# PJLab-ADG/DetZero

Hardware: AMD Instinct MI355X
Metric: LiDAR frames/sec (160k pts, 0.1m voxels) (higher is better)
Workload: dtype f32 as f16 pairs (hi+lo, 22-bit significand; 3 f16 MFMA per product, f32 accumulate)

## Files before the change

### detzero_amd/csrc/conv2d_h.hip

```cpp
#include "hgemm.h"

namespace dz {

int conv3x3_h_variant(const dz_conv2d_desc &p);
int conv3x3_h_launch(const dz_conv2d_desc &p, int bc, int math, int out_f32, size_t w_bytes, hipStream_t stream);

template <class T, class M, bool OUT_F32, int NS>
__global__ __launch_bounds__(256) void k_conv2d_h(dz_conv2d_desc p, long m_total, unsigned int in_bytes, unsigned int w_bytes) {
    extern __shared__ __attribute__((aligned(16))) unsigned char smem_raw[];
    v4u *const smem = reinterpret_cast<v4u *>(smem_raw);
    __shared__ int in_pix[T::BP];
    __shared__ int out_pix[T::BP];
    __shared__ __attribute__((aligned(16))) float sc_s[T::BC], sh_s[T::BC];

    const int tid = threadIdx.x, lane = tid & 63, wid = tid >> 6;
    const int wp = wid / T::WC, wc = wid % T::WC;
    const int ntn = p.cout_pad / T::BC;
    const int nty = ntn * p.groups;
    const int nwg = gridDim.x, q8 = nwg >> 3, r8 = nwg & 7, xcd = blockIdx.x & 7;
    const int lid = (xcd < r8 ? xcd * (q8 + 1) : r8 * (q8 + 1) + (xcd - r8) * q8) + (blockIdx.x >> 3);
    const int by = lid % nty;
    const int grp = by / ntn;
    const int n0 = (by % ntn) * T::BC;
    const long row0 = (long)(lid / nty) * T::BP;
    const bool phases = p.phase_groups != 0;
    const int ph_dy = phases ? grp / p.out_sx : 0, ph_dx = phases ? grp % p.out_sx : 0;
    const int ssg = phases ? 0 : grp;

// ... 163 lines not shown
                }
            }
        }
    }
}

template <class T, class M, bool OUT_F32, int NS>
static int launch_conv_h(const dz_conv2d_desc &p, size_t w_bytes, hipStream_t stream) {
    const long m_total = (long)p.batch * p.ho * p.wo;
    dim3 grid(ceil_div(m_total, T::BP) * (p.cout_pad / T::BC) * p.groups);
    const size_t in_bytes = (size_t)p.batch * p.in_hp * p.in_wp * p.in_cstride * sizeof(float);
    if (in_bytes >= 0x80000000ull || w_bytes >= 0x80000000ull) {
        set_error("dz_conv2d_forward_split: image of %zu bytes / weights of %zu bytes exceed the 2 GiB buffer-addressing limit", in_bytes, w_bytes);
        return DZ_ERR_UNSUPPORTED;
    }
    static PerDeviceFlags lds_done;
    if (int rc_ = reserve_lds(reinterpret_cast<const void *>(&k_conv2d_h<T, M, OUT_F32, NS>), T::LDS_BYTES, lds_done, "dz_conv2d_forward_split")) return rc_;
    hipLaunchKernelGGL((k_conv2d_h<T, M, OUT_F32, NS>), grid, dim3(256), T::LDS_BYTES, stream, p, m_total, (unsigned int)in_bytes,
                       (unsigned int)w_bytes);
    DZ_LAUNCH_CHECK();
    return DZ_OK;
}

enum ConvHVariant { CH_NONE = 0, CH_128_128, CH_128_64, CH_64_128, CH_64_64, CH_128_32, CH_C3_128, CH_C3_64, CH_C3_32 };
static const char *const kConvHVariantName[] = {"none", "k_conv2d_h<128x128x32>", "k_conv2d_h<128x64x32>", "k_conv2d_h<64x128x32>",
                                                "k_conv2d_h<64x64x32>", "k_conv2d_h<128x32x32>", "k_conv3x3_h<8x32x128>",
                                                "k_conv3x3_h<8x32x64>", "k_conv3x3_h<16x32x32>"};

static ConvHVariant conv2d_h_select(const dz_conv2d_desc &p) {
    if (p.cin % 32 != 0) return CH_NONE;
    const long m_total = (long)p.batch * p.ho * p.wo;
    if (p.cout_pad % 64 != 0) return p.cout_pad % 32 == 0 ? CH_128_32 : CH_NONE;
    struct Cand { ConvHVariant v; int bp, bc; double eff; };
    static const Cand cands[4] = {{CH_128_128, 128, 128, 1.00}, {CH_128_64, 128, 64, 0.90}, {CH_64_128, 64, 128, 0.88}, {CH_64_64, 64, 64, 0.78}};
    const int slots = 512;
    double best = -1.0;
    ConvHVariant pick = CH_64_64;
    for (int i = 0; i < 4; ++i) {
        if (p.cout_pad % cands[i].bc != 0) continue;
        const long tiles = (long)ceil_div(m_total, cands[i].bp) * (p.cout_pad / cands[i].bc) * p.groups;
        const long rounds = (tiles + slots - 1) / slots;
        const double useful = (double)m_total / ((double)ceil_div(m_total, cands[i].bp) * cands[i].bp);
        const double score = cands[i].eff * useful * (double)tiles / (double)(rounds * slots);
        if (score > best) { best = score; pick = cands[i].v; }
    }
    return pick;
}

struct ConvHChoice { ConvHVariant v; const char *why; };

static ConvHChoice conv_h_select(const dz_conv2d_desc &p, int out_f32) {
    const int bc3 = conv3x3_h_variant(p);
    if (p.in_rowidx && (!bc3 || out_f32))
        return {CH_NONE, "dz_conv2d_forward_split: in_rowidx (sparse input) is implemented for 3 x 3 stride-1 layers with 128-channel output tiles, "
                         "two z slabs (cin == 2 * in_row_channels) and pair16 output"};
    if (p.in_tiles && bc3 && !((bc3 == 64 || bc3 == 128) && !out_f32))
        return {CH_NONE, "dz_conv2d_forward_split: in_tiles lists 8 x 32 pixel tiles; this layer runs on the 32-channel tile kernel (16 x 32 tiles) - pass no list"};
    if (bc3 && (!out_f32 || bc3 == 32)) return {bc3 == 128 ? CH_C3_128 : bc3 == 64 ? CH_C3_64 : CH_C3_32, nullptr};
    const ConvHVariant v = conv2d_h_select(p);
    return {v, v != CH_NONE ? nullptr : "dz_conv2d_forward_split: unsupported channels cin=%d cout_pad=%d (cin %% 32, cout_pad %% 32 required)"};
}

template <class M, bool OUT_F32>
static int conv2d_h_launch(ConvHVariant v, const dz_conv2d_desc &p, size_t w_bytes, hipStream_t stream) {
    switch (v) {
        case CH_128_128: return launch_conv_h<HTile<128, 128, 32, 2, 2>, M, OUT_F32, 2>(p, w_bytes, stream);
        case CH_128_64: return launch_conv_h<HTile<128, 64, 32, 2, 2>, M, OUT_F32, 3>(p, w_bytes, stream);
        case CH_64_128: return launch_conv_h<HTile<64, 128, 32, 2, 2>, M, OUT_F32, 3>(p, w_bytes, stream);
        case CH_64_64: return launch_conv_h<HTile<64, 64, 32, 2, 2>, M, OUT_F32, 3>(p, w_bytes, stream);
        default: return launch_conv_h<HTile<128, 32, 32, 4, 1>, M, OUT_F32, 3>(p, w_bytes, stream);
    }
}

}

using namespace dz;

extern "C" {

int dz_conv2d_forward_split(const dz_conv2d_desc *d, int math, int out_f32, void *stream_) {
    hipStream_t stream = (hipStream_t)stream_;
// ... 10 lines not shown
        DZ_CHECK_ARG(d->g_cout[g] >= 1 && d->g_cout[g] <= d->cout_pad, "dz_conv2d_forward_split: bad g_cout[%d]", g);
        DZ_CHECK_ARG(out_f32 || (d->g_cout[g] % 8 == 0 && d->g_ooff[g] % 8 == 0),
                     "dz_conv2d_forward_split: pair16 output needs channel counts / offsets in multiples of 8");
    }
    DZ_CHECK_ARG(out_f32 || (d->out_cstride % 8 == 0 && d->out_coff % 8 == 0),
                 "dz_conv2d_forward_split: pair16 output needs channel stride / offset in multiples of 8");
    DZ_CHECK_ARG((d->ho - 1) * d->stride + d->in_off + d->kh - 1 < d->in_hp &&
                 (d->wo - 1) * d->stride + d->in_off + d->kw - 1 < d->in_wp && d->in_off >= 0,
                 "dz_conv2d_forward_split: taps leave the input image");
    DZ_CHECK_ARG(!d->phase_groups || (d->groups == d->out_sy * d->out_sx && d->kh == 1 && d->kw == 1 && d->stride == 1 && !d->group_shift && !d->group_max),
                 "dz_conv2d_forward_split: phase_groups needs groups == out_sy * out_sx (<= 8) and a 1x1 kernel");
    const int ph_y = d->phase_groups ? d->out_sy - 1 : 0, ph_x = d->phase_groups ? d->out_sx - 1 : 0;
    DZ_CHECK_ARG((d->ho - 1) * d->out_sy + d->out_dy + ph_y < d->out_hp && (d->wo - 1) * d->out_sx + d->out_dx + ph_x < d->out_wp,
                 "dz_conv2d_forward_split: output leaves the output image");
    if ((long)d->batch * d->ho * d->wo == 0) return DZ_OK;
    const size_t w_bytes = (size_t)d->groups * d->kh * d->kw * d->cout_pad * d->cin * sizeof(float);
    DZ_CHECK_ARG(!d->in_rowidx || (d->in_row_channels >= 32 && d->in_rows >= 0), "dz_conv2d_forward_split: in_rowidx needs in_row_channels / in_rows");
    const ConvHChoice c = conv_h_select(*d, out_f32);
    switch (c.v) {
        case CH_NONE: set_error(c.why, d->cin, d->cout_pad); return DZ_ERR_UNSUPPORTED;
        case CH_C3_128: return conv3x3_h_launch(*d, 128, math, out_f32, w_bytes, stream);
        case CH_C3_64: return conv3x3_h_launch(*d, 64, math, out_f32, w_bytes, stream);
        case CH_C3_32: return conv3x3_h_launch(*d, 32, math, out_f32, w_bytes, stream);
        default: break;
    }
    if (math == DZ_MATH_F16X2)
        return out_f32 ? conv2d_h_launch<MathF16, true>(c.v, *d, w_bytes, stream) : conv2d_h_launch<MathF16, false>(c.v, *d, w_bytes, stream);
    if (math == DZ_MATH_F16)
        return out_f32 ? conv2d_h_launch<MathF16H, true>(c.v, *d, w_bytes, stream) : conv2d_h_launch<MathF16H, false>(c.v, *d, w_bytes, stream);
    return out_f32 ? conv2d_h_launch<MathBF16, true>(c.v, *d, w_bytes, stream) : conv2d_h_launch<MathBF16, false>(c.v, *d, w_bytes, stream);
}

int dz_linear_forward_split(const float *x, long rows, int cin, int x_stride, const float *w, int cout, int cout_pad, const float *scale,
                            const float *shift, const float *group_shift, int group_rows, int relu, float *y, int y_stride, int math,
                            int out_f32, int group_max, void *stream_) {
    DZ_CHECK_ARG(rows >= 0 && x_stride >= cin && y_stride >= cout && cin % 32 == 0 && cout_pad % 32 == 0 && cout <= cout_pad,
                 "dz_linear_forward_split: bad sizes (cin and cout_pad in multiples of 32)");
    if (group_max) {
        DZ_CHECK_ARG(out_f32 && group_rows >= 128 && group_rows % 128 == 0 && rows % group_rows == 0 && y_stride % 4 == 0 && ((uintptr_t)y & 15u) == 0,
                     "dz_linear_forward_split: group_max needs fp32 output, group_rows %% 128 == 0 (got %d), rows %% group_rows == 0, a 16-byte aligned result", group_rows);
        const long ngroups = rows / group_rows;
        if (y_stride == cout) {
            const int rc = fill_u32(y, 0xFF800000u, (size_t)ngroups * y_stride, (hipStream_t)stream_);
            if (rc) return rc;
        } else {
            for (long g = 0; g < ngroups; ++g) {
// ... 34 lines not shown
```

### detzero_amd/det_modules.py

```python
import collections
import contextlib
import os
from functools import partial

import numpy as np
import torch
import torch.nn as nn

from . import ops, range_audit
from .lib import DetZeroHipError
from .range_audit import RangeAudit

PACKED_TABLES = bool(os.environ.get('DZ_TUNE_PACKED_TABLES'))

K3, S1, P1 = (3, 3, 3), (1, 1, 1), (1, 1, 1)


def _inference_only(module):
    if module.training:
        raise DetZeroHipError('%s: only the inference path is implemented on the HIP backend '
                              '(call .eval()); training is out of scope' % type(module).__name__)


def fold_bn(bn, conv_bias=None):
# ... 684 lines not shown
    return buf


def nchw_to_padded_nhwc(x, pad=1):
    b, c, h, w = x.shape
    out = x.new_zeros((b, h + 2 * pad, w + 2 * pad, c))
    out[:, pad:pad + h, pad:pad + w, :] = x.permute(0, 2, 3, 1)
    return out


def _recode(img, enc, math, e_src=0, e_dst=0):
    if ops.storage_math(enc) == ops.storage_math(math) and e_src == e_dst:
        return img
    plain = ops.pair16_to_f32(img, enc) if enc else img
    if e_src != e_dst:
        plain = plain * (2.0 ** (e_dst - e_src))
    return ops.pair16_from_f32(plain, math=math) if math else plain


SKIP_EMPTY_TILES = os.environ.get('DZ_TUNE_SKIP_EMPTY_TILES', '1') != '0'
SPARSE_BEV_INPUT = os.environ.get('DZ_TUNE_SPARSE_BEV', '1') != '0'
FIRST_BLOCK_WIDE_GROUPS = os.environ.get('DZ_TUNE_FIRST_BLOCK_WIDE', '1') != '0'
FUSED_DEBLOCK_PHASES = os.environ.get('DZ_TUNE_DEBLOCK_PHASES', '1') != '0'


def conv_layer(inp, in_shape, w, scale, shift, relu, out, out_shape, *, cin, in_cstride, in_coff=0, ksize=3,
               stride=1, in_off=0, out_cstride, out_coff=0, out_s=1, out_d=(0, 0), groups=1, cout_pad=None,
               g_cout=None, g_ooff=None, ho=None, wo=None, batch=1, math=0, out_f32=False, phase_groups=False, in_rowidx=None,
               in_row_channels=0, in_rows=0, in_tiles=None, w_limb3=None, w_limb3g=None):
    if cout_pad is None:
        cout_pad = w.shape[-2] if math else w.shape[-1]
    desc = dict(
        inp=inp.data_ptr(), out=out.data_ptr(), w=w.data_ptr(),
        scale=scale.data_ptr() if scale is not None else None,
        shift=shift.data_ptr() if shift is not None else None,
        batch=batch, ho=ho, wo=wo, in_hp=in_shape[0], in_wp=in_shape[1], in_cstride=in_cstride, in_coff=in_coff,
        cin=cin, kh=ksize, kw=ksize, stride=stride, in_off=in_off,
        out_hp=out_shape[0], out_wp=out_shape[1], out_cstride=out_cstride, out_coff=out_coff,
        out_sy=out_s, out_sx=out_s, out_dy=out_d[0], out_dx=out_d[1],
        groups=groups, cout_pad=cout_pad,
        g_cout=g_cout if g_cout is not None else [cout_pad], g_ooff=g_ooff if g_ooff is not None else [0],
        relu=1 if relu else 0, phase_groups=1 if phase_groups else 0,
        in_rowidx=in_rowidx.data_ptr() if in_rowidx is not None else None, in_row_channels=int(in_row_channels), in_rows=int(in_rows),
        in_tiles=in_tiles.data_ptr() if in_tiles is not None else None)
    if w_limb3 is not None and not math and ops.conv3x3_limb3_supported(desc):
        desc['w'] = w_limb3().data_ptr()
# ... 140 lines not shown
                rows, ridx = sparse_in
                wz, scz, shz = self._p(cv, e_in, e_mid, key='w_zmajor')
                conv_layer(rows, (xh + 2, xw + 2), wz, scz, shz, True, y, (oh + 2, ow + 2),
                           cin=cv['cin'], in_cstride=xc, ksize=3, stride=s, in_off=0, out_cstride=cv['cout'],
                           out_d=(1, 1), ho=oh, wo=ow, batch=batch, math=self.math, in_rowidx=ridx, in_row_channels=rows.shape[1],
                           in_rows=rows.shape[0], in_tiles=tiles[0] if tiles is not None else None)
                if tiles is not None:
                    ops.bev_fill_empty_tiles(tiles[0], batch, oh, ow, shz, True, cv['cout'], y, self.math)
            else:
                tl = tiles[ci] if (tiles is not None and ci < tiles.shape[0]) else None
                wc, scc, shc = self._p(cv, e_in if (li == 0 and ci == 0) else e_mid, e_mid)
                conv_layer(x, (xh + 2, xw + 2), wc, scc, shc, True, y, (oh + 2, ow + 2),
                           cin=cv['cin'], in_cstride=xc, ksize=3, stride=s, in_off=0, out_cstride=cv['cout'],
                           out_d=(1, 1), ho=oh, wo=ow, batch=batch, math=self.math, in_tiles=tl, w_limb3=self._l3(cv),
                           w_limb3g=self._l3g(cv))
                if tl is not None:
                    ops.bev_fill_empty_tiles(tl, batch, oh, ow, shc, True, cv['cout'], y, self.math, zero_resp=zero[ci])
            if audit is not None:
                audit.probe('backbone2d.blocks.%d.%d' % (li, 1 + 3 * ci), y, math=self.math, stage='spatial_features_2d', exp=e_mid)
            x, xh, xw, xc = y, oh, ow, cv['cout']
        return x, xh, xw, xc

    def _level_deblock(self, lvl, x, xh, xw, xc, concat, coff, h, w, batch, li=0):
        self._deblock_launches(lvl, x, xh, xw, xc, concat, coff, h, w, batch)
        de = lvl['de']
        audit = range_audit.active()
        if audit is not None:
            audit.probe('backbone2d.deblocks.%d' % li, concat, math=self.math, stage='spatial_features_2d', exp=self._e('spatial_features_2d'),
                        c_off=coff, c=de['cout'])
        return coff + de['cout']

    def _deblock_launches(self, lvl, x, xh, xw, xc, concat, coff, h, w, batch):
        de = lvl['de']
        s = de['s']
        ctot = self.num_bev_features
        e_mid = self._e('spatial_features_2d')
        if xh * s != h or xw * s != w:
            raise DetZeroHipError('BaseBEVBackbone: deblock output %dx%d does not match %dx%d' % (xh * s, xw * s, h, w))
        if self.math and 1 < s * s <= 8 and FUSED_DEBLOCK_PHASES:
            conv_layer(x, (xh + 2, xw + 2), *self._p(de, e_mid, e_mid, key='w_phases'), True, concat,
                       (h + 2, w + 2), cin=de['cin'], in_cstride=xc, ksize=1, stride=1, in_off=1,
                       out_cstride=ctot, out_coff=coff, out_s=s, out_d=(1, 1), ho=xh, wo=xw, batch=batch, math=self.math,
                       groups=s * s, g_cout=[de['cout']] * (s * s), g_ooff=[0] * (s * s), phase_groups=True)
            return
        for dy in range(s):
            for dx in range(s):
                conv_layer(x, (xh + 2, xw + 2), *self._p(de['phases'][dy][dx], e_mid, e_mid, scale=de['scale'], shift=de['shift']), True, concat,
# ... 440 lines not shown
```

### detzero_amd/lib.py

```python
import ctypes
import os

import torch

_HERE = os.path.dirname(os.path.abspath(__file__))
LIB_PATH = os.path.join(_HERE, 'libdetzero_hip.so')


ERR_INVALID, ERR_WORKSPACE, ERR_HIP, ERR_UNSUPPORTED = -1, -2, -3, -4


class DetZeroHipError(RuntimeError):
    pass


c_int, c_float, c_size_t, c_void_p, c_double = ctypes.c_int, ctypes.c_float, ctypes.c_size_t, ctypes.c_void_p, ctypes.c_double
c_longlong = ctypes.c_longlong
_I3 = c_int * 3
_F3 = c_float * 3
_F6 = c_float * 6
_I8 = c_int * 8


class Conv2dDesc(ctypes.Structure):
    _fields_ = [
        ('inp', c_void_p), ('out', c_void_p), ('w', c_void_p), ('scale', c_void_p), ('shift', c_void_p),
        ('batch', c_int), ('ho', c_int), ('wo', c_int),
        ('in_hp', c_int), ('in_wp', c_int), ('in_cstride', c_int), ('in_coff', c_int), ('cin', c_int),
        ('kh', c_int), ('kw', c_int), ('stride', c_int), ('in_off', c_int),
        ('out_hp', c_int), ('out_wp', c_int), ('out_cstride', c_int), ('out_coff', c_int),
        ('out_sy', c_int), ('out_sx', c_int), ('out_dy', c_int), ('out_dx', c_int),
        ('groups', c_int), ('cout_pad', c_int),
        ('g_cout', _I8), ('g_ooff', _I8),
        ('relu', c_int),
        ('group_shift', c_void_p), ('group_rows', c_int), ('group_max', c_int), ('phase_groups', c_int),
        ('in_rowidx', c_void_p), ('in_row_channels', c_int), ('in_rows', c_int), ('in_tiles', c_void_p),
    ]


class TrackTable(ctypes.Structure):
    _fields_ = [(k, c_void_p) for k in ('x', 'P', 'Q', 'dt', 'box', 'cls', 'score', 'update_score', 'num_points', 'hit', 'miss', 'id')] + [('cap', c_int)]


class TrackAb3d(ctypes.Structure):
    _fields_ = [(k, c_void_p) for k in ('x', 'P', 'box', 'work', 'hits')] + [('stride', c_int)]


_TT = ctypes.POINTER(TrackTable)
_TA = ctypes.POINTER(TrackAb3d)
_F8 = c_float * 8


class TrackSeqParams(ctypes.Structure):
    _fields_ = [(k, c_int) for k in ('metric', 'distinguish_class', 'gate_class', 'n_cls', 'two_stage', 'merge_enable', 'death_age',
                                     'init_track_id')] + \
               [(k, _F8) for k in ('thr_first', 'thr_second', 'thr_merge')] + [(k, c_float) for k in ('p0', 'p1', 'q0', 'q1', 'r', 'dt')] + \
               [(k, c_int) for k in ('filter', 'birth_age')]


# ... 94 lines not shown
                                          c_void_p, c_int, c_void_p, c_int, c_void_p]),
    'dz_spconv_x_limb3_window_rows': (c_int, [c_int, c_int]),
    'dz_spconv_x_limb3_variant': (ctypes.c_char_p, [c_int, c_int]),
    'dz_spconv_forward_limb3': (c_int, [c_void_p, c_int, c_int, c_void_p, c_void_p, c_int, c_int, c_void_p, c_void_p, c_void_p, c_void_p,
                                        c_void_p, c_int, c_void_p, c_int, c_void_p]),
    'dz_spconv_limb3_tile_rows': (c_int, [c_int, c_int]),
    'dz_spconv_limb3_variant': (ctypes.c_char_p, [c_int, c_int]),
    'dz_spconv_forward_limb3_w': (c_int, [c_void_p, c_int, c_int, c_void_p, c_void_p, c_int, c_int, c_void_p, c_void_p, c_void_p, c_void_p,
                                          c_void_p, c_int, c_void_p, c_int, c_int, c_void_p]),
    'dz_spconv_limb3_w_tile_rows': (c_int, [c_int, c_int]),
    'dz_spconv_limb3_w_variant': (ctypes.c_char_p, [c_int, c_int]),
    'dz_bev_tile_cover_words': (c_size_t, [c_int, c_int, c_int]),
    'dz_bev_tile_cover_offset': (c_size_t, [c_int, c_int, c_int]),
    'dz_bev_tile_cover_ws_words': (c_size_t, [c_int, c_int, c_int, c_int]),
    'dz_bev_tile_cover': (c_int, [c_void_p, c_int, c_int, c_int, c_int, c_int, c_int, c_void_p, c_void_p, c_void_p]),
    'dz_bev_fill_spans': (c_int, [c_void_p, c_int, c_int, c_int, c_void_p, c_int, c_int, c_void_p, c_int, c_int, c_int, c_int, c_void_p, c_int, c_void_p]),
    'dz_bev_row_index': (c_int, [c_void_p, c_void_p, c_int, c_int, c_int, c_int, c_int, c_int, c_int, c_void_p, c_void_p]),
    'dz_sparse_to_bev_split': (c_int, [c_void_p, c_void_p, c_void_p, c_int, c_int, c_int, c_int, c_int, c_int, c_void_p,
                                       c_void_p]),
    'dz_sparse_to_bev_split_dense': (c_int, [c_void_p, c_int, c_void_p, c_void_p, c_int, c_int, c_int, c_int, c_int, c_int, c_int, c_void_p,
                                             c_void_p]),
    'dz_conv2d_forward_split': (c_int, [ctypes.POINTER(Conv2dDesc), c_int, c_int, c_void_p]),
    'dz_conv2d_variant_split': (ctypes.c_char_p, [ctypes.POINTER(Conv2dDesc), c_int]),
    'dz_conv3x3_limb3_forward': (c_int, [ctypes.POINTER(Conv2dDesc), c_void_p]),
    'dz_conv3x3_limb3_supported': (c_int, [ctypes.POINTER(Conv2dDesc)]),
    'dz_conv3x3_limb3_variant': (ctypes.c_char_p, [ctypes.POINTER(Conv2dDesc)]),
    'dz_conv2d_limb3_forward': (c_int, [ctypes.POINTER(Conv2dDesc), c_void_p]),
    'dz_conv2d_limb3_supported': (c_int, [ctypes.POINTER(Conv2dDesc)]),
    'dz_conv2d_limb3_variant': (ctypes.c_char_p, [ctypes.POINTER(Conv2dDesc)]),
    'dz_spconv_variant_split': (ctypes.c_char_p, [c_int, c_int]),
    'dz_spconv_variant_split_arm': (ctypes.c_char_p, [c_int, c_int, c_int, c_int, c_size_t]),
    'dz_spconv_variant_split_packed': (ctypes.c_char_p, [c_int, c_int]),
    'dz_xattn_folded_supported': (c_int, [c_int, c_int, c_int]),
    'dz_xattn_folded_workspace_bytes': (ctypes.c_size_t, [c_int, c_int]),
    'dz_xattn_folded': (c_int, [c_void_p] * 6 + [c_int] * 5 + [ctypes.c_float, c_void_p, ctypes.c_size_t, c_void_p, c_void_p]),
    'dz_roi_bev_features': (c_int, [c_void_p, c_int, c_void_p, ctypes.c_long, ctypes.c_long, c_int, c_int, c_int] + [ctypes.c_float] * 4 + [c_int, c_void_p, c_void_p]),
    'dz_linear_splitk_workspace_bytes': (ctypes.c_size_t, [c_int, c_int, c_int]),
    'dz_linear_forward_splitk': (c_int, [c_void_p, c_int, c_int, c_int, c_void_p, c_int, c_int, c_void_p, c_void_p, c_int, c_void_p, c_int, c_int, c_void_p,
                                         ctypes.c_size_t, c_void_p]),
    'dz_mha_core_split': (c_int, [c_void_p, c_void_p, c_void_p, c_void_p, c_int, c_int, c_int, c_int, ctypes.c_float, c_void_p, c_int, c_void_p]),
    'dz_mha_core_limb3': (c_int, [c_void_p, c_void_p, c_void_p, c_void_p, c_int, c_int, c_int, c_int, ctypes.c_float, c_void_p, c_void_p]),
    'dz_mha_core_limb3_supported': (c_int, [c_int, c_int, c_int, c_int]),
    'dz_pdv_sa_pool_supported': (c_int, [c_int] * 7),
    'dz_pdv_sa_pool': (c_int, [c_void_p, c_int, c_int, c_void_p, c_void_p, c_int, c_void_p, c_void_p, c_int, c_void_p, c_void_p, c_int,
                               c_void_p, c_int, c_void_p, c_void_p, c_int, c_void_p, c_int, c_void_p, c_void_p, c_int, c_int, c_void_p, c_void_p]),
    'dz_pdv_encoder_front': (c_int, [c_void_p, c_int, c_void_p, c_void_p, ctypes.c_long] + [c_void_p] * 9 + [c_int, c_void_p]),
# ... 175 lines not shown
```

### detzero_amd/ops.py

```python
import ctypes
import os
from typing import Callable, NamedTuple, Optional

import numpy as np
import torch

from . import lib as L


def _dev():
    return torch.device('cuda', torch.cuda.current_device())


def _ws(nbytes):
    return torch.empty((max(int(nbytes), 256),), dtype=torch.uint8, device=_dev())


def grid_size_of(pc_range, voxel_size):
    r = np.asarray(pc_range, dtype=np.float32)
    return np.round((r[3:6] - r[0:3]) / np.array(voxel_size)).astype(np.int64)


def voxelize_hard_nosync(points, pc_range, voxel_size, max_points, max_voxels, xy_range_mask=False):
    lib = L.load()
# ... 645 lines not shown
        raise L.DetZeroHipError('range_probe: %d rows asked of a tensor of %d' % (rows, cap))
    c = stride - int(c_off) if c is None else int(c)
    L.check(lib.dz_range_probe(L.ptr(t) if rows else None, rows, L.ptr(d_rows), stride, int(c_off), c, storage_math(math_id(math)), L.ptr(slot_view),
                               L.stream()), 'dz_range_probe')


def range_reset(table):
    L.require_cuda(table)
    L.check(L.load().dz_range_reset(L.ptr(table), table.shape[0], L.stream()), 'dz_range_reset')


def range_read(table):
    raw = table.cpu().numpy().view(np.uint64).reshape(-1, 4)
    out = np.zeros((raw.shape[0],), dtype=RANGE_DTYPE)
    out['peak'] = (raw[:, 0] & np.uint64(0xFFFFFFFF)).astype(np.uint32).view(np.float32)
    out['saturated'], out['nonfinite'], out['elements'] = raw[:, 1], raw[:, 2], raw[:, 3]
    return out


DENSE_F32_ENGINES = ('mfma32', 'bf16x3')
DENSE_F32_GENERIC_ENGINES = ('mfma32', 'bf16x3')


def _conv2d_desc(desc_kwargs):
    d = L.Conv2dDesc()
    for k, v in desc_kwargs.items():
        if k in ('g_cout', 'g_ooff'):
            arr = getattr(d, k)
            for i, e in enumerate(v):
                arr[i] = int(e)
        else:
            setattr(d, k, v)
    return d


def conv3x3_limb3_supported(desc_kwargs):
    return bool(L.load().dz_conv3x3_limb3_supported(ctypes.byref(_conv2d_desc(desc_kwargs))))


def conv2d_limb3_supported(desc_kwargs):
    return bool(L.load().dz_conv2d_limb3_supported(ctypes.byref(_conv2d_desc(desc_kwargs))))


def pack_weight_limb3_generic(w):
    return pack_weight_limb3(w.reshape(-1, w.shape[-2], w.shape[-1]), cout_mult=32)


def conv2d(desc_kwargs, math=0, out_f32=False, tiles=None, f32_engine=None, f32_generic=None):
    lib = L.load()
    if f32_engine not in (None,) + DENSE_F32_ENGINES:
        raise L.DetZeroHipError('unknown fp32 dense engine %r (%s)' % (f32_engine, ' | '.join(DENSE_F32_ENGINES)))
    if f32_generic not in (None,) + DENSE_F32_GENERIC_ENGINES:
        raise L.DetZeroHipError('unknown generic fp32 dense engine %r (%s)' % (f32_generic, ' | '.join(DENSE_F32_GENERIC_ENGINES)))
    limb3 = f32_engine == 'bf16x3' and not math
    limb3g = f32_generic == 'bf16x3' and not math and not limb3
    d = _conv2d_desc(desc_kwargs)

    def launch():
        if limb3:
            L.check(lib.dz_conv3x3_limb3_forward(ctypes.byref(d), L.stream()), 'dz_conv3x3_limb3_forward')
        elif limb3g:
            L.check(lib.dz_conv2d_limb3_forward(ctypes.byref(d), L.stream()), 'dz_conv2d_limb3_forward')
        elif math:
            L.check(lib.dz_conv2d_forward_split(ctypes.byref(d), int(math), 1 if out_f32 else 0, L.stream()), 'dz_conv2d_forward_split')
        else:
            L.check(lib.dz_conv2d_forward(ctypes.byref(d), L.stream()), 'dz_conv2d_forward')
    if PROFILER is None:
        launch()
        return
    m = d.batch * d.ho * d.wo
    taps = d.kh * d.kw
    cout = sum(d.g_cout[i] for i in range(d.groups))
    flops = 2.0 * m * taps * d.cin * cout
    nbytes = 4.0 * (m * d.cin * (1 if d.phase_groups else d.groups) + m * cout + taps * d.cin * d.cout_pad * d.groups)
    if tiles is not None:
        share = int(tiles[0]) / float(max(d.batch * (-(-d.ho // 8)) * (-(-d.wo // 32)), 1))
        flops *= share
        nbytes = 4.0 * (share * (m * d.cin + m * cout) + taps * d.cin * d.cout_pad * d.groups)
    if limb3:
# ... 1321 lines not shown
```

### include/detzero_hip.h

```cpp
#ifndef DETZERO_HIP_H
#define DETZERO_HIP_H

#include <stddef.h>
#include <stdint.h>

#ifdef __cplusplus
extern "C" {
#endif

#define DZ_OK 0
#define DZ_ERR_INVALID (-1)
#define DZ_ERR_WORKSPACE (-2)
#define DZ_ERR_HIP (-3)
#define DZ_ERR_UNSUPPORTED (-4)

const char *dz_version(void);
const char *dz_last_error(void);
int dz_device_cu_count(void);


size_t dz_voxelize_hard_workspace_bytes(int n, int gx, int gy, int gz, int max_points);
int dz_voxelize_hard(const float *points, int n, int c, const float *h_range6, const float *h_vsize3,
                     const int *h_grid3, int xy_range_mask, int max_points, int max_voxels, float *voxels,
                     int *coords_zyx, int *num_points, int *d_num_voxels, void *ws, size_t ws_bytes,
// ... 56 lines not shown

typedef struct dz_conv2d_desc {
    const float *in;
    float *out;
    const float *w;
    const float *scale;
    const float *shift;
    int batch, ho, wo;
    int in_hp, in_wp, in_cstride, in_coff, cin;
    int kh, kw, stride, in_off;
    int out_hp, out_wp, out_cstride, out_coff;
    int out_sy, out_sx, out_dy, out_dx;
    int groups, cout_pad;
    int g_cout[8];
    int g_ooff[8];
    int relu;
    const float *group_shift;
    int group_rows;
    int group_max;
    int phase_groups;
    const int *in_rowidx;
    int in_row_channels, in_rows;
    const int *in_tiles;
} dz_conv2d_desc;
int dz_conv2d_forward(const dz_conv2d_desc *h_desc, void *stream);
const char *dz_conv2d_variant(const dz_conv2d_desc *h_desc);
const char *dz_spconv_variant(int cin, int cout);

#define DZ_MATH_F32 0
#define DZ_MATH_F16X2 1
#define DZ_MATH_BF16X2 2
#define DZ_MATH_F16 3
int dz_pair16_from_f32(const float *src, long rows, int c_src, int c_dst, int math, float *dst, void *stream);
int dz_pair16_to_f32(const float *src, long rows, int c, int math, float *dst, void *stream);
int dz_range_probe(const float *x, long rows, const int *d_rows, int row_stride_words, int c_off, int c, int math, unsigned long long *slot,
                   void *stream);
int dz_range_reset(unsigned long long *table, int n_slots, void *stream);
int dz_scatter_rows_split(const float *src, const int *rank, const int *d_n, int n_cap, int c_src, float *dst,
                          int c_dst, int math, void *stream);
int dz_spconv_forward_split(const float *in, int in_rows, int cin, const int *nbr, const uint32_t *tile_masks, int kvol,
                            int cap_out, const int *d_m_out, const float *w, const float *scale, const float *shift,
                            const float *residual, int relu, float *out, int cout, int math, void *stream);
int dz_spconv_tile_rows(void);
int dz_spconv_tile_info_words(void);
int dz_spconv_tile_table_entries(void);
size_t dz_build_tiles_halo_stride(int kvol);
// ... 33 lines not shown
                            const int *d_m_out, const float *w_limb, const float *scale, const float *shift, const float *residual,
                            int relu, float *out, int cout, void *stream);
int dz_spconv_limb3_tile_rows(int cin, int cout);
const char *dz_spconv_limb3_variant(int cin, int cout);
int dz_spconv_forward_limb3_w(const float *in, int in_rows, int cin, const int *nbr, const uint32_t *tile_masks, int kvol, int cap_out,
                              const int *d_m_out, const float *w_limb, const float *scale, const float *shift, const float *residual,
                              int relu, float *out, int cout, int max_workgroups, void *stream);
int dz_spconv_limb3_w_tile_rows(int cin, int cout);
const char *dz_spconv_limb3_w_variant(int cin, int cout);
int dz_bev_row_index(const uint32_t *bitmap, const uint32_t *prefix, int batch, int d, int h, int w, int layout, int pad, int feat_rows,
                     int *idx, void *stream);
size_t dz_bev_tile_cover_words(int batch, int ho, int wo);
size_t dz_bev_tile_cover_offset(int batch, int ho, int wo);
size_t dz_bev_tile_cover_ws_words(int batch, int ho, int wo, int nlists);
int dz_bev_tile_cover(const int *idx, int batch, int hp, int wp, int ho, int wo, int nlists, int *lists, int *ws, void *stream);
int dz_bev_fill_spans(const int *list, int batch, int ho, int wo, const float *shift, int relu, int cout, float *out, int out_hp, int out_wp,
                      int out_cstride, int out_coff, const float *zero_resp, int math, void *stream);
int dz_sparse_to_bev_split(const float *feats, const int *coords, const int *d_m, int cap, int c, int d, int h,
                           int w, int pad, float *bev, void *stream);
int dz_sparse_to_bev_split_dense(const float *feats, int feat_rows, const uint32_t *bitmap, const uint32_t *prefix, int batch, int c,
                                 int d, int h, int w, int layout, int pad, float *bev, void *stream);
int dz_conv2d_forward_split(const dz_conv2d_desc *h_desc, int math, int out_f32, void *stream);
const char *dz_conv2d_variant_split(const dz_conv2d_desc *h_desc, int out_f32);
int dz_conv3x3_limb3_forward(const dz_conv2d_desc *h_desc, void *stream);
int dz_conv3x3_limb3_supported(const dz_conv2d_desc *h_desc);
const char *dz_conv3x3_limb3_variant(const dz_conv2d_desc *h_desc);
int dz_conv2d_limb3_forward(const dz_conv2d_desc *h_desc, void *stream);
int dz_conv2d_limb3_supported(const dz_conv2d_desc *h_desc);
const char *dz_conv2d_limb3_variant(const dz_conv2d_desc *h_desc);
int dz_linear_forward_split(const float *x, long rows, int cin, int x_stride, const float *w, int cout, int cout_pad, const float *scale,
                            const float *shift, const float *group_shift, int group_rows, int relu, float *y, int y_stride, int math,
                            int out_f32, int group_max, void *stream);
const char *dz_spconv_variant_split(int cin, int cout);
const char *dz_spconv_variant_split_arm(int cin, int cout, int kvol, int has_tile_masks, size_t nbr_bytes);
const char *dz_spconv_variant_split_packed(int cin, int cout);
int dz_xattn_folded_supported(int lq, int e, int heads);
size_t dz_xattn_folded_workspace_bytes(int b, int lk);
int dz_xattn_folded(const float *q, const float *mem, const uint8_t *key_padding_mask, const float *wk_oi, const float *wv_io, const float *bv,
                    int b, int lq, int lk, int e, int heads, float scale, float *workspace, size_t workspace_bytes, float *out, void *stream);
int dz_mlp_chain_forward(const float *x, long rows, const float *wa, const float *sa, const float *ba, const float *group_shift, int ldg, int group_rows,
                         const float *wb, const float *sb, const float *bb, const float *wk, const float *bk, const float *wv, const float *bv,
                         float *mem, float *k, float *v, int math, void *stream);
int dz_pointnet3_forward(const float *x, long rows, const float *w1, const float *s1, const float *b1, const float *w2, const float *s2,
                         const float *b2, const float *w3, const float *s3, const float *b3, int c3, int group_rows, float *tap, float *out,
                         int x_cols_f32, int math, void *stream);

// ... 333 lines not shown
```

Baseline: 1162.

## Add persistent streaming 1x1 deblock kernel with cross-tile pipelined epilogue

Adds a persistent k_deblock_h kernel (256x128x32 tiles, 512 threads) for the 1x1 phase-grouped deblock convolutions. Each workgroup walks a band of pixel tiles assigned per XCD and keeps a 3-stage load pipeline running across tile boundaries. The epilogue's split-f16 output stores go out through buffer stores and are covered by counted vmcnt waits instead of a full drain. A stream_1x1 flag is added to the descriptor and set via a Python context manager around the deblock launches. The aim is to remove per-tile launch, prologue and epilogue stalls. The cost is a small fixed grid, 32 slots per XCD, which may leave CUs idle, plus hand-tuned wait counts that must stay exact.

Measured after the change: 1169 (median of 6 runs). No clear change (+0.6%).

```diff
diff --git a/detzero_amd/csrc/conv2d_h.hip b/detzero_amd/csrc/conv2d_h.hip
--- a/detzero_amd/csrc/conv2d_h.hip
+++ b/detzero_amd/csrc/conv2d_h.hip
@@ -4,6 +4,8 @@
 
 int conv3x3_h_variant(const dz_conv2d_desc &p);
 int conv3x3_h_launch(const dz_conv2d_desc &p, int bc, int math, int out_f32, size_t w_bytes, hipStream_t stream);
+int deblock_h_variant(const dz_conv2d_desc &p);
+int deblock_h_launch(const dz_conv2d_desc &p, int math, hipStream_t stream);
 
 template <class T, class M, bool OUT_F32, int NS>
 __global__ __launch_bounds__(256) void k_conv2d_h(dz_conv2d_desc p, long m_total, unsigned int in_bytes, unsigned int w_bytes) {
@@ -213,10 +215,10 @@
     return DZ_OK;
 }
 
-enum ConvHVariant { CH_NONE = 0, CH_128_128, CH_128_64, CH_64_128, CH_64_64, CH_128_32, CH_C3_128, CH_C3_64, CH_C3_32 };
+enum ConvHVariant { CH_NONE = 0, CH_128_128, CH_128_64, CH_64_128, CH_64_64, CH_128_32, CH_C3_128, CH_C3_64, CH_C3_32, CH_DEBLOCK };
 static const char *const kConvHVariantName[] = {"none", "k_conv2d_h<128x128x32>", "k_conv2d_h<128x64x32>", "k_conv2d_h<64x128x32>",
                                                 "k_conv2d_h<64x64x32>", "k_conv2d_h<128x32x32>", "k_conv3x3_h<8x32x128>",
-                                                "k_conv3x3_h<8x32x64>", "k_conv3x3_h<16x32x32>"};
+                                                "k_conv3x3_h<8x32x64>", "k_conv3x3_h<16x32x32>", "k_deblock_h<256x128x32>"};
 
 static ConvHVariant conv2d_h_select(const dz_conv2d_desc &p) {
     if (p.cin % 32 != 0) return CH_NONE;
@@ -248,6 +250,7 @@
     if (p.in_tiles && bc3 && !((bc3 == 64 || bc3 == 128) && !out_f32))
         return {CH_NONE, "dz_conv2d_forward_split: in_tiles lists 8 x 32 pixel tiles; this layer runs on the 32-channel tile kernel (16 x 32 tiles) - pass no list"};
     if (bc3 && (!out_f32 || bc3 == 32)) return {bc3 == 128 ? CH_C3_128 : bc3 == 64 ? CH_C3_64 : CH_C3_32, nullptr};
+    if (p.stream_1x1 && !out_f32 && !bc3 && deblock_h_variant(p)) return {CH_DEBLOCK, nullptr};
     const ConvHVariant v = conv2d_h_select(p);
     return {v, v != CH_NONE ? nullptr : "dz_conv2d_forward_split: unsupported channels cin=%d cout_pad=%d (cin %% 32, cout_pad %% 32 required)"};
 }
@@ -304,6 +307,7 @@
         case CH_C3_128: return conv3x3_h_launch(*d, 128, math, out_f32, w_bytes, stream);
         case CH_C3_64: return conv3x3_h_launch(*d, 64, math, out_f32, w_bytes, stream);
         case CH_C3_32: return conv3x3_h_launch(*d, 32, math, out_f32, w_bytes, stream);
+        case CH_DEBLOCK: return deblock_h_launch(*d, math, stream);
         default: break;
     }
     if (math == DZ_MATH_F16X2)
diff --git a/detzero_amd/csrc/deblock_h.hip b/detzero_amd/csrc/deblock_h.hip
--- /dev/null
+++ b/detzero_amd/csrc/deblock_h.hip
@@ -0,0 +1,286 @@
+#include "hgemm.h"
+
+namespace dz {
+
+using DbTile = HTile<256, 128, 32, 4, 2>;
+constexpr int DB_NS = 3;
+constexpr int DB_NST = DbTile::P_PER_THREAD + DbTile::C_PER_THREAD;
+constexpr int DB_EPI_STORES = DbTile::PT * DbTile::CT * 2 * 2;
+constexpr int DB_LDS_STG = DbTile::LDS_BYTES;
+constexpr int DB_LDS_SC = DB_LDS_STG + (DbTile::THREADS / 64) * STG_WAVE_BYTES;
+constexpr int DB_LDS_BYTES = DB_LDS_SC + 2 * DbTile::BC * 4;
+static_assert(DB_LDS_BYTES <= 160 * 1024, "does not fit the LDS of a CU");
+static_assert((DB_NS - 1) * DB_NST + DB_NS * DB_EPI_STORES < 64, "the largest counted wait must fit the 6 bits of vmcnt");
+
+template <int N>
+__device__ __forceinline__ void db_wait_vm() {
+    asm volatile("s_waitcnt vmcnt(%0)" ::"n"(N));
+}
+
+__device__ __forceinline__ void db_store16(v4u d, unsigned int voff, __amdgpu_buffer_rsrc_t rsrc) {
+    __builtin_amdgcn_raw_buffer_store_b128(d, rsrc, (int)voff, 0, 0);
+}
+
+__device__ __forceinline__ void db_barrier() {
+    asm volatile("s_waitcnt lgkmcnt(0)" ::: "memory");
+    __builtin_amdgcn_s_barrier();
+    asm volatile("" ::: "memory");
+}
+
+template <class M>
+__global__ __launch_bounds__(DbTile::THREADS) void k_deblock_h(dz_conv2d_desc p, int m_total, int npx, unsigned int in_bytes,
+                                                                unsigned int w_bytes, unsigned int out_bytes) {
+    using T = DbTile;
+    extern __shared__ __attribute__((aligned(16))) unsigned char smem_raw[];
+    v4u *const smem = reinterpret_cast<v4u *>(smem_raw);
+    v4u *const Ps0 = smem, *const Cs0 = smem + 2 * T::PS_U4;
+    float *const sc_s = reinterpret_cast<float *>(smem_raw + DB_LDS_SC), *const sh_s = sc_s + T::BC;
+
+    const int tid = threadIdx.x, lane = tid & 63, wid = tid >> 6;
+    const int wp = wid / T::WC, wc = wid % T::WC;
+    const int ntn = p.cout_pad / T::BC, nty = ntn * p.groups;
+    const int xcd = blockIdx.x & 7, jloc = blockIdx.x >> 3, nj = gridDim.x >> 3;
+    const int grp = (jloc % nty) / ntn;
+    const int n0 = ((jloc % nty) % ntn) * T::BC;
+    const int band_lo = (int)((long)xcd * npx >> 3), band_hi = (int)((long)(xcd + 1) * npx >> 3);
+    const int tstep = nj / nty;
+    const int tile0 = band_lo + jloc / nty;
+    if (jloc / nty >= tstep || tile0 >= band_hi) return;
+    const int nk = p.cin / T::KC;
+    const int nchunks = ((band_hi - tile0 + tstep - 1) / tstep) * nk;
+
+    const bool phases = p.phase_groups != 0;
+    const int ph_dy = phases ? grp / p.out_sx : 0, ph_dx = phases ? grp % p.out_sx : 0;
+    const int ooff = p.out_coff + p.g_ooff[grp];
+    const bool relu = p.relu != 0;
+
+    if (tid < T::BC) {
+        sc_s[tid] = p.scale ? p.scale[n0 + tid] : 1.f;
+        sh_s[tid] = p.shift ? p.shift[n0 + tid] : 0.f;
+    }
+
+    const srsrc_t prsrc = make_srsrc(p.in, in_bytes);
+    const srsrc_t crsrc = make_srsrc(p.w, w_bytes);
+    const __amdgpu_buffer_rsrc_t orsrc = __builtin_amdgcn_make_buffer_rsrc(p.out, 0, (int)out_bytes, 0x00020000);
+
+    auto in_pixel = [&](int m) __attribute__((always_inline)) {
+        if (m >= m_total) return -1;
+        const unsigned int t = (unsigned int)m / (unsigned int)p.wo, x = (unsigned int)m - t * p.wo;
+        const unsigned int b = t / (unsigned int)p.ho, y = t - b * p.ho;
+        return (int)((b * p.in_hp + y + p.in_off) * p.in_wp + x + p.in_off);
+    };
+    auto out_pixel = [&](int m) __attribute__((always_inline)) {
+        if (m >= m_total) return -1;
+        const unsigned int t = (unsigned int)m / (unsigned int)p.wo, x = (unsigned int)m - t * p.wo;
+        const unsigned int b = t / (unsigned int)p.ho, y = t - b * p.ho;
+        return (int)((b * p.out_hp + y * p.out_sy + p.out_dy + ph_dy) * p.out_wp + x * p.out_sx + p.out_dx + ph_dx);
+    };
+
+    unsigned int pvoff[T::P_PER_THREAD], cvoff[T::C_PER_THREAD];
+    const int prow = tid / (T::KC / 4), pq = tid % (T::KC / 4);
+    auto pixel_offsets = [&](int tile) __attribute__((always_inline)) {
+#pragma unroll
+        for (int i = 0; i < T::P_PER_THREAD; ++i) {
+            const int ip = tile < band_hi ? in_pixel(tile * T::BP + prow + i * (T::THREADS / (T::KC / 4))) : -1;
+            pvoff[i] = ip >= 0 ? (unsigned int)(((long)ip * p.in_cstride + p.in_coff + pq * 4) * 4) : OOB_OFFSET;
+        }
+    };
+#pragma unroll
+    for (int i = 0; i < T::C_PER_THREAD; ++i) {
+        const int idx = tid + i * T::THREADS;
+        cvoff[i] = (unsigned int)((((long)grp * p.cout_pad + n0 + idx / (T::KC / 4)) * p.cin + (idx % (T::KC / 4)) * 4) * 4);
+    }
+    int itile = tile0, ikc = 0;
+    pixel_offsets(itile);
+    auto issue = [&](HStage<T> &st) __attribute__((always_inline)) {
+        const unsigned int add = (unsigned int)(ikc * T::KC * 4);
+        const bool live = itile < band_hi;
+#pragma unroll
+        for (int i = 0; i < T::P_PER_THREAD; ++i)
+            asm volatile("buffer_load_dwordx4 %0, %1, %2, 0 offen" : "=v"(st.p[i]) : "v"(pvoff[i] + add), "s"(prsrc));
+#pragma unroll
+        for (int i = 0; i < T::C_PER_THREAD; ++i)
+            asm volatile("buffer_load_dwordx4 %0, %1, %2, 0 offen" : "=v"(st.c[i]) : "v"(live ? cvoff[i] + add : OOB_OFFSET), "s"(crsrc));
+        if (++ikc == nk) {
+            ikc = 0;
+            if (live) {
+                itile += tstep;
+                pixel_offsets(itile);
+            }
+        }
+    };
+
+    f32x16 acc[T::CT][T::PT];
+#pragma unroll
+    for (int i = 0; i < T::CT; ++i)
+#pragma unroll
+        for (int j = 0; j < T::PT; ++j)
+#pragma unroll
+            for (int e = 0; e < 16; ++e) acc[i][j][e] = 0.f;
+
+    unsigned char *const stg = smem_raw + DB_LDS_STG + wid * STG_WAVE_BYTES;
+    auto epilogue = [&](int tile) __attribute__((always_inline)) {
+        const int g = lane & 3, h = lane >> 5;
+        unsigned int orow[T::PT][2];
+#pragma unroll
+        for (int pt = 0; pt < T::PT; ++pt)
+#pragma unroll
+            for (int i = 0; i < 2; ++i) {
+                const int op = out_pixel(tile * T::BP + wp * T::PT * 32 + pt * 32 + (lane >> 2) + 16 * i);
+                orow[pt][i] = op >= 0 ? (unsigned int)(((long)op * p.out_cstride + ooff) * 4) : OOB_OFFSET;
+            }
+#pragma unroll
+        for (int pt = 0; pt < T::PT; ++pt) {
+#pragma unroll
+            for (int ct = 0; ct < T::CT; ++ct) {
+#pragma unroll
+                for (int j = 0; j < 4; ++j) {
+                    const float4 v = make_float4(acc[ct][pt][4 * j], acc[ct][pt][4 * j + 1], acc[ct][pt][4 * j + 2], acc[ct][pt][4 * j + 3]);
+                    *reinterpret_cast<float4 *>(stg + (lane & 31) * STG_ROW_BYTES + j * 32 + h * 16) = v;
+                }
+                __builtin_amdgcn_fence(__ATOMIC_RELEASE, "wavefront");
+                __builtin_amdgcn_wave_barrier();
+                __builtin_amdgcn_fence(__ATOMIC_ACQUIRE, "wavefront");
+                const int lc = wc * T::CT * 32 + ct * 32 + g * 8;
+                const float4 sc0 = *reinterpret_cast<const float4 *>(sc_s + lc), sc1 = *reinterpret_cast<const float4 *>(sc_s + lc + 4);
+                const float4 sh0 = *reinterpret_cast<const float4 *>(sh_s + lc), sh1 = *reinterpret_cast<const float4 *>(sh_s + lc + 4);
+                float4 va[2], vb[2];
+#pragma unroll
+                for (int i = 0; i < 2; ++i) {
+                    const int r = (lane >> 2) + 16 * i;
+                    va[i] = *reinterpret_cast<const float4 *>(stg + r * STG_ROW_BYTES + g * 32);
+                    vb[i] = *reinterpret_cast<const float4 *>(stg + r * STG_ROW_BYTES + g * 32 + 16);
+                }
+#pragma unroll
+                for (int i = 0; i < 2; ++i) {
+                    float v[8] = {fmaf(va[i].x, sc0.x, sh0.x), fmaf(va[i].y, sc0.y, sh0.y), fmaf(va[i].z, sc0.z, sh0.z), fmaf(va[i].w, sc0.w, sh0.w),
+                                  fmaf(vb[i].x, sc1.x, sh1.x), fmaf(vb[i].y, sc1.y, sh1.y), fmaf(vb[i].z, sc1.z, sh1.z), fmaf(vb[i].w, sc1.w, sh1.w)};
+                    if (relu) {
+#pragma unroll
+                        for (int e = 0; e < 8; ++e) v[e] = fmaxf(v[e], 0.f);
+                    }
+                    const float v0[4] = {v[0], v[1], v[2], v[3]}, v1[4] = {v[4], v[5], v[6], v[7]};
+                    uint2 h0, l0, h1, l1;
+                    split4<M>(v0, h0, l0);
+                    split4<M>(v1, h1, l1);
+                    const unsigned int off = orow[pt][i] == OOB_OFFSET ? OOB_OFFSET : orow[pt][i] + (unsigned int)((n0 + lc) * 4);
+                    db_store16(v4u{h0.x, h0.y, h1.x, h1.y}, off, orsrc);
+                    db_store16(v4u{l0.x, l0.y, l1.x, l1.y}, off + 16u, orsrc);
+                }
+                __builtin_amdgcn_fence(__ATOMIC_RELEASE, "wavefront");
+                __builtin_amdgcn_wave_barrier();
+                __builtin_amdgcn_fence(__ATOMIC_ACQUIRE, "wavefront");
+            }
+        }
+    };
+
+    HStage<T> st[DB_NS];
+    issue(st[0]);
+    wait_hstage<T, 0>(st[0]);
+    store_hstage<T>(st[0], Ps0, Cs0, tid);
+    __syncthreads();
+    issue(st[1 % DB_NS]);
+    issue(st[2 % DB_NS]);
+    issue(st[3 % DB_NS]);
+
+    const int poff = (wp * T::PT * 32 + (lane & 31)) * T::ROW_U4 + (lane >> 5) * 2;
+    const int coff = (wc * T::CT * 32 + (lane & 31)) * T::ROW_U4 + (lane >> 5) * 2;
+    HFrag<T> f0, f1;
+    load_hfrag<T>(f0, Ps0 + poff, Cs0 + coff, 0);
+
+    int ctile = tile0, ckc = 0;
+    unsigned int ehist = 0u;
+    auto body = [&](int c, auto s_t) __attribute__((always_inline)) {
+        constexpr int S = decltype(s_t)::value;
+        const int cur = c & 1;
+        const v4u *Pc = Ps0 + cur * T::PS_U4 + poff, *Cc = Cs0 + cur * T::CS_U4 + coff;
+        const v4u *Pn = Ps0 + (cur ^ 1) * T::PS_U4 + poff, *Cn = Cs0 + (cur ^ 1) * T::CS_U4 + coff;
+        load_hfrag<T>(f1, Pc, Cc, 1);
+        constexpr int L = (DB_NS - 1) * DB_NST, E = DB_EPI_STORES;
+        switch (__builtin_popcount(ehist)) {
+            case 0: db_wait_vm<L>(); break;
+            case 1: db_wait_vm<L + E>(); break;
+            case 2: db_wait_vm<L + 2 * E>(); break;
+            default: db_wait_vm<L + 3 * E>(); break;
+        }
+#pragma unroll
+        for (int i = 0; i < T::P_PER_THREAD; ++i) asm volatile("" : "+v"(st[S].p[i]));
+#pragma unroll
+        for (int i = 0; i < T::C_PER_THREAD; ++i) asm volatile("" : "+v"(st[S].c[i]));
+        store_hstage<T>(st[S], Ps0 + (cur ^ 1) * T::PS_U4, Cs0 + (cur ^ 1) * T::CS_U4, tid);
+        __builtin_amdgcn_sched_barrier(0);
+        mma_hfrag<T, M>(f0, acc);
+        __builtin_amdgcn_sched_barrier(0);
+        db_barrier();
+        load_hfrag<T>(f0, Pn, Cn, 0);
+        issue(st[S]);
+        __builtin_amdgcn_sched_barrier(0);
+        mma_hfrag<T, M>(f1, acc);
+        __builtin_amdgcn_sched_barrier(0);
+        const bool last = ++ckc == nk;
+        if (last) {
+            epilogue(ctile);
+            ckc = 0;
+            ctile += tstep;
+#pragma unroll
+            for (int i = 0; i < T::CT; ++i)
+#pragma unroll
+                for (int j = 0; j < T::PT; ++j)
+#pragma unroll
+                    for (int e = 0; e < 16; ++e) acc[i][j][e] = 0.f;
+        }
+        ehist = ((ehist << 1) | (last ? 1u : 0u)) & ((1u << DB_NS) - 1u);
+    };
+    static_assert(DB_NS == 3, "the trip below is unrolled for three stages");
+    for (int c = 0; c < nchunks; c += DB_NS) {
+        body(c, std::integral_constant<int, 1>{});
+        if (c + 1 < nchunks) body(c + 1, std::integral_constant<int, 2>{});
+        if (c + 2 < nchunks) body(c + 2, std::integral_constant<int, 0>{});
+    }
+    asm volatile("s_waitcnt vmcnt(0)");
+}
+
+int deblock_h_variant(const dz_conv2d_desc &p) {
+    if (p.kh != 1 || p.kw != 1 || p.stride != 1) return 0;
+    if (p.groups < 1 || p.groups > 8 || (p.groups != 1 && !p.phase_groups)) return 0;
+    if (p.phase_groups && (p.out_sy < 1 || p.out_sx < 1 || p.groups != p.out_sy * p.out_sx)) return 0;
+    if (p.cin < DbTile::KC || p.cin % DbTile::KC != 0 || p.cout_pad < DbTile::BC || p.cout_pad % DbTile::BC != 0) return 0;
+    for (int g = 0; g < p.groups; ++g)
+        if (p.g_cout[g] != p.cout_pad) return 0;
+    if (p.in_rowidx || p.in_tiles || p.group_shift || p.group_max) return 0;
+    if (p.batch < 1 || p.ho < 1 || p.wo < 1) return 0;
+    const size_t in_bytes = (size_t)p.batch * p.in_hp * p.in_wp * p.in_cstride * sizeof(float);
+    const size_t out_bytes = (size_t)p.batch * p.out_hp * p.out_wp * p.out_cstride * sizeof(float);
+    const size_t w_bytes = (size_t)p.groups * p.cout_pad * p.cin * sizeof(float);
+    if (in_bytes >= 0x80000000ull || out_bytes >= 0x80000000ull || w_bytes >= 0x80000000ull) return 0;
+    return DbTile::BC;
+}
+
+template <class M>
+static int launch_deblock(const dz_conv2d_desc &p, hipStream_t stream) {
+    using T = DbTile;
+    const long m_total = (long)p.batch * p.ho * p.wo;
+    const int npx = ceil_div(m_total, T::BP);
+    const size_t in_bytes = (size_t)p.batch * p.in_hp * p.in_wp * p.in_cstride * sizeof(float);
+    const size_t out_bytes = (size_t)p.batch * p.out_hp * p.out_wp * p.out_cstride * sizeof(float);
+    const size_t w_bytes = (size_t)p.groups * p.cout_pad * p.cin * sizeof(float);
+    static PerDeviceFlags lds_done;
+    if (int rc_ = reserve_lds(reinterpret_cast<const void *>(&k_deblock_h<M>), DB_LDS_BYTES, lds_done, "dz_conv2d_forward_split")) return rc_;
+    const int nty = p.cout_pad / T::BC * p.groups;
+    const int slots = 32;
+    const int per_xcd = slots / nty * nty < nty ? nty : slots / nty * nty;
+    hipLaunchKernelGGL((k_deblock_h<M>), dim3(8u * per_xcd), dim3(T::THREADS), DB_LDS_BYTES, stream, p, (int)m_total, npx,
+                       (unsigned int)in_bytes, (unsigned int)w_bytes, (unsigned int)out_bytes);
+    DZ_LAUNCH_CHECK();
+    return DZ_OK;
+}
+
+int deblock_h_launch(const dz_conv2d_desc &p, int math, hipStream_t stream) {
+    if (math == DZ_MATH_F16X2) return launch_deblock<MathF16>(p, stream);
+    if (math == DZ_MATH_F16) return launch_deblock<MathF16H>(p, stream);
+    return launch_deblock<MathBF16>(p, stream);
+}
+
+}
+
+extern "C" int dz_deblock_h_variant(const dz_conv2d_desc *d) { return d ? dz::deblock_h_variant(*d) : 0; }
diff --git a/detzero_amd/det_modules.py b/detzero_amd/det_modules.py
--- a/detzero_amd/det_modules.py
+++ b/detzero_amd/det_modules.py
@@ -730,6 +730,7 @@
 SPARSE_BEV_INPUT = os.environ.get('DZ_TUNE_SPARSE_BEV', '1') != '0'
 FIRST_BLOCK_WIDE_GROUPS = os.environ.get('DZ_TUNE_FIRST_BLOCK_WIDE', '1') != '0'
 FUSED_DEBLOCK_PHASES = os.environ.get('DZ_TUNE_DEBLOCK_PHASES', '1') != '0'
+STREAM_DEBLOCKS = True
 
 
 def conv_layer(inp, in_shape, w, scale, shift, relu, out, out_shape, *, cin, in_cstride, in_coff=0, ksize=3,
@@ -916,7 +917,8 @@
         return x, xh, xw, xc
 
     def _level_deblock(self, lvl, x, xh, xw, xc, concat, coff, h, w, batch, li=0):
-        self._deblock_launches(lvl, x, xh, xw, xc, concat, coff, h, w, batch)
+        with ops.stream_1x1(STREAM_DEBLOCKS):
+            self._deblock_launches(lvl, x, xh, xw, xc, concat, coff, h, w, batch)
         de = lvl['de']
         audit = range_audit.active()
         if audit is not None:
diff --git a/detzero_amd/lib.py b/detzero_amd/lib.py
--- a/detzero_amd/lib.py
+++ b/detzero_amd/lib.py
@@ -35,6 +35,7 @@
         ('relu', c_int),
         ('group_shift', c_void_p), ('group_rows', c_int), ('group_max', c_int), ('phase_groups', c_int),
         ('in_rowidx', c_void_p), ('in_row_channels', c_int), ('in_rows', c_int), ('in_tiles', c_void_p),
+        ('stream_1x1', c_int),
     ]
 
 
@@ -175,6 +176,7 @@
                                              c_void_p]),
     'dz_conv2d_forward_split': (c_int, [ctypes.POINTER(Conv2dDesc), c_int, c_int, c_void_p]),
     'dz_conv2d_variant_split': (ctypes.c_char_p, [ctypes.POINTER(Conv2dDesc), c_int]),
+    'dz_deblock_h_variant': (c_int, [ctypes.POINTER(Conv2dDesc)]),
     'dz_conv3x3_limb3_forward': (c_int, [ctypes.POINTER(Conv2dDesc), c_void_p]),
     'dz_conv3x3_limb3_supported': (c_int, [ctypes.POINTER(Conv2dDesc)]),
     'dz_conv3x3_limb3_variant': (ctypes.c_char_p, [ctypes.POINTER(Conv2dDesc)]),
diff --git a/detzero_amd/ops.py b/detzero_amd/ops.py
--- a/detzero_amd/ops.py
+++ b/detzero_amd/ops.py
@@ -1,5 +1,7 @@
+import contextlib
 import ctypes
 import os
+import threading
 from typing import Callable, NamedTuple, Optional
 
 import numpy as np
@@ -691,6 +693,23 @@
 DENSE_F32_GENERIC_ENGINES = ('mfma32', 'bf16x3')
 
 
+_ROUTE = threading.local()
+
+
+@contextlib.contextmanager
+def stream_1x1(on=True):
+    prev = getattr(_ROUTE, 'stream_1x1', False)
+    _ROUTE.stream_1x1 = bool(on)
+    try:
+        yield
+    finally:
+        _ROUTE.stream_1x1 = prev
+
+
+def deblock_stream_supported(desc_kwargs):
+    return bool(L.load().dz_deblock_h_variant(ctypes.byref(_conv2d_desc(desc_kwargs))))
+
+
 def _conv2d_desc(desc_kwargs):
     d = L.Conv2dDesc()
     for k, v in desc_kwargs.items():
@@ -724,6 +743,8 @@
     limb3 = f32_engine == 'bf16x3' and not math
     limb3g = f32_generic == 'bf16x3' and not math and not limb3
     d = _conv2d_desc(desc_kwargs)
+    if math and getattr(_ROUTE, 'stream_1x1', False):
+        d.stream_1x1 = 1
 
     def launch():
         if limb3:
diff --git a/include/detzero_hip.h b/include/detzero_hip.h
--- a/include/detzero_hip.h
+++ b/include/detzero_hip.h
@@ -102,6 +102,7 @@
     const int *in_rowidx;
     int in_row_channels, in_rows;
     const int *in_tiles;
+    int stream_1x1;
 } dz_conv2d_desc;
 int dz_conv2d_forward(const dz_conv2d_desc *h_desc, void *stream);
 const char *dz_conv2d_variant(const dz_conv2d_desc *h_desc);
@@ -181,6 +182,7 @@
                                  int d, int h, int w, int layout, int pad, float *bev, void *stream);
 int dz_conv2d_forward_split(const dz_conv2d_desc *h_desc, int math, int out_f32, void *stream);
 const char *dz_conv2d_variant_split(const dz_conv2d_desc *h_desc, int out_f32);
+int dz_deblock_h_variant(const dz_conv2d_desc *h_desc);
 int dz_conv3x3_limb3_forward(const dz_conv2d_desc *h_desc, void *stream);
 int dz_conv3x3_limb3_supported(const dz_conv2d_desc *h_desc);
 const char *dz_conv3x3_limb3_variant(const dz_conv2d_desc *h_desc);
```
